# mjq11302010044/TPGSR

Hardware: AMD Instinct MI355X
Metric: training img/s (16x64->32x128, bs=48/GPU), TPGSR-TSRN full train step (higher is better)
Workload: dtype bf16x2; 1 GPU; C3: TPGSR-TSRN = TSRN_TL (STN+mask) + CRNN teacher/student text prior, stu_iter 1, full train step (teacher fwd, student fwd+bwd, distill loss, prior dropout, SR fwd+bwd, ImageLoss(gradient), clip 0.25, Adam); tpg=crnn, batch_per_gpu=48, global_batch=48, parallelism=dp1, launch=recorded plans, plain launches: main + weight-gradient + teacher streams

## Files before the change

include/tpgsr_hip.h:

```cpp
#ifndef TPGSR_HIP_H
#define TPGSR_HIP_H

#ifdef __cplusplus
extern "C" {
#endif

#define TPGSR_ACT_NONE 0
#define TPGSR_ACT_RELU 1
#define TPGSR_ACT_MISH 2
#define TPGSR_ACT_TANH 3
#define TPGSR_ACT_PRELU 4

const char* tpgsr_last_error(void);
int tpgsr_version(void);
int tpgsr_sizeof(int which);

typedef struct {
  const float* in;
  const float* in2;
  const float* in_scale;
  const float* in_shift;
  const float* wt;
  const float* bias;
  float* out;
// ... 252 lines not shown
  const float* dghn;
  const float* h;
  float* partC;
  float* dbC;
  float* partH;
  float* dbH;
  int axis;
  int zsplits;
} tpgsr_gru_wgrad_args;
int tpgsr_gru_wgrad_splits(long long P);
int tpgsr_gru_wgrad(const tpgsr_gru_wgrad_args* w, void* stream);
void tpgsr_gru_set_prefetch(int steps);

int tpgsr_tps_grid_fwd(const float* ctrl, const float* inv_kernel, const float* coord_repr, int N, int HW,
                       int NC, float* grid, float* src, void* stream);
int tpgsr_tps_grid_bwd(const float* dgrid, const float* src, const float* inv_kernel, const float* coord_repr,
                       int N, int HW, int NC, float* dctrl, void* stream);
int tpgsr_grid_sample_fwd(const float* in, const float* grid, int N, int H, int W, int C, int OH, int OW,
                          int align_corners, float* out, void* stream);
int tpgsr_grid_sample_bwd(const float* in, const float* grid, const float* dout, int N, int H, int W, int C,
                          int OH, int OW, int align_corners, float* din ,
                          float* dgrid , void* stream);

int tpgsr_strip_resample_fwd(const float* in, const float* scale, const float* shift, int act, int N, int Win, int Wout,
                             int C, float* out, void* stream);
int tpgsr_strip_resample_bwd(const float* in, const float* scale, const float* shift, int act, const float* dout, int N,
                             int Win, int Wout, int C, float* dz, void* stream);
int tpgsr_hsum(const float* d, int N, int H, int W, int C, float* dstrip, int accumulate, void* stream);

int tpgsr_bicubic_gray_fwd(const float* in_nchw, int N, int Ctot, int H, int W, int OH, int OW, float* out, void* stream);
int tpgsr_bicubic_gray_bwd(const float* dout, int N, int Ctot, int H, int W, int OH, int OW, float* din_nchw, void* stream);
int tpgsr_im2col3x3_c1(const float* in, int N, int H, int W, float* col , void* stream);
int tpgsr_col2im3x3_c1(const float* dcol, int N, int H, int W, float* din, void* stream);
int tpgsr_pad_channels(const float* src, long long M, int Cs, int Cd, float* dst, void* stream);
int tpgsr_pool2d_fwd(const float* x, int N, int H, int W, int C, const float* scale, const float* shift, int act, int KH,
                     int KW, int SH, int SW, int PH, int PW, float* out, void* stream);
int tpgsr_pool2d_bwd(const float* x, const float* dout, int N, int H, int W, int C, const float* scale, const float* shift,
                     int act, int KH, int KW, int SH, int SW, int PH, int PW, float* dz, void* stream);
int tpgsr_lstm_rec_gemm(const float* a0, const float* a1, long long a_stride, const float* b0, const float* b1, int Nrows,
                        int K, int Nc, int S, float* out, void* stream);
int tpgsr_lstm_step_fwd(float* G, const float* gh, int nsplit, const float* bhh , float* Cst, float* out,
                        int N, int T, int Hh, int step, void* stream);
int tpgsr_lstm_seq_fwd(float* G, const float* whhT, const float* bhh, float* Cst, float* out, void* hx, unsigned* sync, int N, int T,
                       int Hh, void* stream);
long long tpgsr_lstm_seq_hx_bytes(void);
int tpgsr_lstm_seq_probe(unsigned* words, void* stream);
int tpgsr_lstm_seq_fwdg(float* G, const float* whhT, const float* bhh, float* Cst, float* out, void* hg, unsigned* sync, int N, int T,
                        int Hh, void* stream);
long long tpgsr_lstm_seq_hg_bytes(void);
int tpgsr_lstm_seq_bwd(float* G, const float* Cst, const float* dout, const float* w0, const float* w1, void* px, unsigned* sync, int N,
                       int T, int Hh, void* stream);
long long tpgsr_lstm_seq_px_bytes(void);
int tpgsr_lstm_step_bwd(float* G, const float* Cst, const float* dout, const float* dhc, int nsplit, float* dcc, int N, int T,
                        int Hh, int step, void* stream);
int tpgsr_softmax_prior_fwd(const float* logits, const float* q, int N, int T, int C, int drop_n, float* p, float* prior_nchw,
                            float* partial, int nblk, void* stream);
int tpgsr_semantic_loss_finalize(const float* partial, int nblk, long long count, float w, float* loss, void* stream);
int tpgsr_softmax_prior_bwd(const float* p, const float* q, const float* dprior_nchw, const float* dp_in, int N, int T, int C,
                            int drop_n, float wsem, float* dlogits, int nblk, void* stream);
int tpgsr_ctc_loss(const float* logits, int sn, int st, const int* targets, const int* tgt_off, const int* tgt_len, const float* weight,
                   int N, int T, int C, int blank, float scale, float* nll, float* dlogits, int accumulate, int max_len, void* stream);
int tpgsr_semantic_loss_fwd(const float* p, const float* q, long long n, float* partial, int nblk, void* stream);
int tpgsr_semantic_loss_bwd(const float* p, const float* q, const float* dloss, long long n, float* dp, void* stream);

int tpgsr_copy_strided(const float* src, int src_ld, int src_coff, float* dst, int dst_ld, int dst_coff, long long M, int C,
                       int accumulate, void* stream);
// ... 98 lines not shown
```

tpgsr_amd/csrc/crnn.hip:

```cpp
#include "common.h"
#include "gru_common.h"
#include <stdlib.h>

__device__ __forceinline__ void cubic_coeffs(float t, float (&w)[4]) {
  const float A = -0.75f;
  float x = t + 1.f;
  w[0] = ((A * x - 5.f * A) * x + 8.f * A) * x - 4.f * A;
  x = t;
  w[1] = ((A + 2.f) * x - (A + 3.f)) * x * x + 1.f;
  x = 1.f - t;
  w[2] = ((A + 2.f) * x - (A + 3.f)) * x * x + 1.f;
  x = 2.f - t;
  w[3] = ((A * x - 5.f * A) * x + 8.f * A) * x - 4.f * A;
}

__device__ __forceinline__ void bicubic_src(int o, int in_size, int out_size, int& i0, float (&w)[4]) {
  float scale = (float)in_size / (float)out_size;
  float x = ((float)o + 0.5f) * scale - 0.5f;
  float fx = floorf(x);
  i0 = (int)fx;
  cubic_coeffs(x - fx, w);
}
__device__ __forceinline__ int clampi(int v, int lo, int hi) { return v < lo ? lo : (v > hi ? hi : v); }

// ... 412 lines not shown

extern "C" int tpgsr_pool2d_bwd(const float* x, const float* dout, int N, int H, int W, int C, const float* scale, const float* shift,
                                int act, int KH, int KW, int SH, int SW, int PH, int PW, float* dz, void* stream) {
  TPGSR_CHECK_ARG(x && dout && dz && KH > 0 && KW > 0 && SH > 0 && SW > 0, "tpgsr_pool2d_bwd: bad arguments");
  int OH = (H + 2 * PH - KH) / SH + 1, OW = (W + 2 * PW - KW) / SW + 1;
  const bool vec = (C & 3) == 0 && ((((uintptr_t)x | (uintptr_t)dout | (uintptr_t)dz) & 15) == 0);
  long long total = (long long)N * H * W * (vec ? C / 4 : C);
  TPGSR_CHECK_ARG((long long)N * H * W * C < (1ll << 31), "tpgsr_pool2d_bwd: map too large for the kernels' 32-bit indices");
  int grid = (int)min((long long)16384, (total + 255) / 256);
  static const bool fast2x2 = [] { const char* e = getenv("TPGSR_POOL2X2_FAST"); return !(e && e[0] == '0'); }();
  if (fast2x2 && vec && KH == 2 && KW == 2 && SH == 2 && SW == 2 && PH == 0 && PW == 0 && !(H & 1) && !(W & 1) &&
      (!scale || !(((uintptr_t)scale | (uintptr_t)shift) & 15))) {
    const long long tw = (long long)N * (H / 2) * (W / 2) * (C / 4);
    hipLaunchKernelGGL(pool2x2_bwd_kernel, dim3((int)min((long long)16384, (tw + 255) / 256)), dim3(256), 0, (hipStream_t)stream, x, dout, N, H, W,
                       C, scale, shift, act, dz);
    TPGSR_LAUNCH_CHECK("tpgsr_pool2d_bwd");
  }
  if (fast2x2 && vec && KH == 2 && KW == 2 && SH == 2 && SW == 1 && PH == 0 && PW == 1 && !(H & 1) &&
      (!scale || !(((uintptr_t)scale | (uintptr_t)shift) & 15))) {
    const long long tw = (long long)N * (H / 2) * W * (C / 4);
    hipLaunchKernelGGL(pool2x2s21_bwd_kernel, dim3((int)min((long long)16384, (tw + 255) / 256)), dim3(256), 0, (hipStream_t)stream, x, dout, N, H,
                       W, C, scale, shift, act, dz);
    TPGSR_LAUNCH_CHECK("tpgsr_pool2d_bwd");
  }
  if (vec)
    hipLaunchKernelGGL(pool2d_bwd_kernel<4>, dim3(grid), dim3(256), 0, (hipStream_t)stream, x, dout, N, H, W, C, scale, shift, act, KH, KW,
                       SH, SW, PH, PW, OH, OW, dz);
  else
    hipLaunchKernelGGL(pool2d_bwd_kernel<1>, dim3(grid), dim3(256), 0, (hipStream_t)stream, x, dout, N, H, W, C, scale, shift, act, KH, KW,
                       SH, SW, PH, PW, OH, OW, dz);
  TPGSR_LAUNCH_CHECK("tpgsr_pool2d_bwd");
}

#define RG_KC 32
__global__ __launch_bounds__(256) void lstm_rec_gemm_kernel(const float* __restrict__ a0, const float* __restrict__ a1,
                                                            long long a_stride, const float* __restrict__ b0,
                                                            const float* __restrict__ b1, int Nrows, int K, int Nc, int S,
                                                            float* __restrict__ out) {
  __shared__ float As[RG_KC][65];
  __shared__ float Bs[RG_KC][64];
  const int d = blockIdx.z, sp = blockIdx.y, n0 = blockIdx.x * 64;
  const float* A = d == 0 ? a0 : a1;
  const float* B = d == 0 ? b0 : b1;
  const int tid = threadIdx.x, lane = tid & 63, wave = tid >> 6;
  const int wm = wave & 1, wn = wave >> 1;
  const int kper = (K / RG_KC + S - 1) / S * RG_KC;
  const int kbeg = sp * kper, kend = min(K, kbeg + kper);
  const int aq = tid & 7, am0 = tid >> 3, bk0 = tid >> 4, bc = (tid & 15) * 4;
  floatx16 acc;
#pragma unroll
  for (int i = 0; i < 16; ++i) acc[i] = 0.f;
  const int arow = lane >> 5, acol = wm * 32 + (lane & 31), bcol = wn * 32 + (lane & 31);
  for (int k0 = kbeg; k0 < kend; k0 += RG_KC) {
    float4 ra0 = make_float4(0.f, 0.f, 0.f, 0.f), ra1 = ra0;
    const int k = k0 + aq * 4;
    if (am0 < Nrows && k < kend) ra0 = *reinterpret_cast<const float4*>(A + (size_t)am0 * a_stride + k);
    if (am0 + 32 < Nrows && k < kend) ra1 = *reinterpret_cast<const float4*>(A + (size_t)(am0 + 32) * a_stride + k);
    float4 rb0 = make_float4(0.f, 0.f, 0.f, 0.f), rb1 = rb0;
    if (k0 + bk0 < kend) rb0 = *reinterpret_cast<const float4*>(B + (size_t)(k0 + bk0) * Nc + n0 + bc);
    if (k0 + bk0 + 16 < kend) rb1 = *reinterpret_cast<const float4*>(B + (size_t)(k0 + bk0 + 16) * Nc + n0 + bc);
    __syncthreads();
    As[aq * 4 + 0][am0] = ra0.x; As[aq * 4 + 1][am0] = ra0.y; As[aq * 4 + 2][am0] = ra0.z; As[aq * 4 + 3][am0] = ra0.w;
    As[aq * 4 + 0][am0 + 32] = ra1.x; As[aq * 4 + 1][am0 + 32] = ra1.y; As[aq * 4 + 2][am0 + 32] = ra1.z; As[aq * 4 + 3][am0 + 32] = ra1.w;
    *reinterpret_cast<float4*>(&Bs[bk0][bc]) = rb0;
    *reinterpret_cast<float4*>(&Bs[bk0 + 16][bc]) = rb1;
    __syncthreads();
// ... 368 lines not shown
```

tpgsr_amd/csrc/plan.cpp:

```cpp
#include <hip/hip_runtime.h>
#include <string.h>
#include <memory>
#include <string>
#include <tuple>
#include <type_traits>
#include <unordered_map>
#include <utility>
#include <vector>
#include "../../include/tpgsr_hip.h"

void tpgsr_set_error(const char* fmt, ...);

namespace {

typedef int (*thunk_fn)(const tpgsr_plan_arg* a, void* stream);

template <typename T>
inline T arg_as(const tpgsr_plan_arg& a) {
  if constexpr (std::is_pointer<T>::value) return reinterpret_cast<T>(const_cast<void*>(a.p));
  else if constexpr (std::is_floating_point<T>::value) return static_cast<T>(a.f);
  else return static_cast<T>(a.i);
}

template <typename Tuple, typename F, size_t... I>
// ... 13 lines not shown
    return call_with<Tuple>(fn, a, st, std::make_index_sequence<sizeof...(P) - 1>{});
  }
};

struct Entry {
  thunk_fn fn;
  int nargs;
  int struct_bytes;
};

#define TPGSR_REG(sym) {#sym, {&Thunk<decltype(&sym), &sym>::call, Thunk<decltype(&sym), &sym>::nargs, 0}}
#define TPGSR_REG_S(sym, T) {#sym, {&Thunk<decltype(&sym), &sym>::call, Thunk<decltype(&sym), &sym>::nargs, (int)sizeof(T)}}

const std::unordered_map<std::string, Entry>& registry() {
  static const std::unordered_map<std::string, Entry> r = {
      TPGSR_REG_S(tpgsr_conv_fwd, tpgsr_conv_args), TPGSR_REG_S(tpgsr_conv_wgrad, tpgsr_wgrad_args),
      TPGSR_REG(tpgsr_wgrad_reduce), TPGSR_REG(tpgsr_wgrad_reduce_program), TPGSR_REG(tpgsr_conv_wgrad_batch), TPGSR_REG(tpgsr_compose_bwd_program), TPGSR_REG(tpgsr_pack_conv_weight), TPGSR_REG(tpgsr_pack_tail_weight),
      TPGSR_REG(tpgsr_pack_program), TPGSR_REG(tpgsr_mfma_probe), TPGSR_REG(tpgsr_copy), TPGSR_REG(tpgsr_zero),
      TPGSR_REG(tpgsr_bn_finalize), TPGSR_REG(tpgsr_bn_stats), TPGSR_REG(tpgsr_bn_bwd_reduce),
      TPGSR_REG(tpgsr_bn_bwd_finalize), TPGSR_REG(tpgsr_bn_bwd_apply), TPGSR_REG(tpgsr_affine_act),
      TPGSR_REG(tpgsr_affine_act_pool), TPGSR_REG(tpgsr_affine_act_pool_bwd), TPGSR_REG(tpgsr_prelu_fwd),
      TPGSR_REG(tpgsr_prelu_bwd), TPGSR_REG(tpgsr_add), TPGSR_REG(tpgsr_add_n), TPGSR_REG(tpgsr_act_bwd), TPGSR_REG(tpgsr_nchw_to_nhwc),
      TPGSR_REG(tpgsr_nhwc_to_nchw), TPGSR_REG(tpgsr_reduce_partials), TPGSR_REG(tpgsr_bigru_fwd),
      TPGSR_REG(tpgsr_bigru_bwd), TPGSR_REG(tpgsr_bigru_bwd2), TPGSR_REG(tpgsr_bigru_fwd_u), TPGSR_REG(tpgsr_bigru_bwd_u), TPGSR_REG_S(tpgsr_bigru_proj_fwd, tpgsr_bigru_proj_args), TPGSR_REG_S(tpgsr_gru_wgrad, tpgsr_gru_wgrad_args), TPGSR_REG(tpgsr_tps_grid_fwd), TPGSR_REG(tpgsr_tps_grid_bwd),
      TPGSR_REG(tpgsr_grid_sample_fwd), TPGSR_REG(tpgsr_grid_sample_bwd), TPGSR_REG(tpgsr_strip_resample_fwd),
      TPGSR_REG(tpgsr_strip_resample_bwd), TPGSR_REG(tpgsr_hsum), TPGSR_REG(tpgsr_bicubic_gray_fwd),
      TPGSR_REG(tpgsr_bicubic_gray_bwd), TPGSR_REG(tpgsr_pool2d_fwd), TPGSR_REG(tpgsr_pool2d_bwd),
      TPGSR_REG(tpgsr_lstm_rec_gemm), TPGSR_REG(tpgsr_lstm_step_fwd), TPGSR_REG(tpgsr_lstm_seq_fwd), TPGSR_REG(tpgsr_lstm_seq_fwdg), TPGSR_REG(tpgsr_lstm_seq_bwd), TPGSR_REG(tpgsr_lstm_step_bwd), TPGSR_REG(tpgsr_softmax_prior_fwd),
      TPGSR_REG(tpgsr_semantic_loss_finalize), TPGSR_REG(tpgsr_softmax_prior_bwd), TPGSR_REG(tpgsr_tail_shiftsum_tanh), TPGSR_REG(tpgsr_shiftsum_nhwc),
      TPGSR_REG(tpgsr_tail_bwd), TPGSR_REG(tpgsr_image_loss_fwd), TPGSR_REG(tpgsr_image_loss_finalize),
      TPGSR_REG(tpgsr_image_loss_bwd), TPGSR_REG(tpgsr_l1_loss_fwd), TPGSR_REG(tpgsr_l1_loss_bwd), TPGSR_REG(tpgsr_sumsq_partial), TPGSR_REG(tpgsr_clip_coef),
      TPGSR_REG(tpgsr_adam_step), TPGSR_REG(tpgsr_step_inc), TPGSR_REG(tpgsr_scale_),
      TPGSR_REG(tpgsr_im2col3x3_c1), TPGSR_REG(tpgsr_col2im3x3_c1), TPGSR_REG(tpgsr_pad_channels),
      TPGSR_REG(tpgsr_semantic_loss_fwd), TPGSR_REG(tpgsr_semantic_loss_bwd), TPGSR_REG(tpgsr_split_bf_program),
      TPGSR_REG(tpgsr_copy_strided), TPGSR_REG(tpgsr_resize_nearest_fwd), TPGSR_REG(tpgsr_resize_nearest_bwd), TPGSR_REG(tpgsr_resize_bilinear_fwd),
      TPGSR_REG(tpgsr_resize_bilinear_bwd), TPGSR_REG(tpgsr_dilate2d), TPGSR_REG(tpgsr_subsample2d), TPGSR_REG(tpgsr_hreduce), TPGSR_REG(tpgsr_hbroadcast),
      TPGSR_REG(tpgsr_bicubic_upsample),
      TPGSR_REG(tpgsr_tconv4s2_expand), TPGSR_REG(tpgsr_tconv4s2_fold_grad), TPGSR_REG(tpgsr_tconv4s2_small_fwd),
      TPGSR_REG(tpgsr_tconv4s2_small_bwd_data), TPGSR_REG(tpgsr_tconv4s2_small_bwd_weight), TPGSR_REG(tpgsr_leaky_relu_fwd),
      TPGSR_REG(tpgsr_leaky_relu_bwd), TPGSR_REG(tpgsr_charbonnier_loss_fwd), TPGSR_REG(tpgsr_charbonnier_loss_bwd),
      TPGSR_REG(tpgsr_leaky_relu_window), TPGSR_REG(tpgsr_scaled_add), TPGSR_REG(tpgsr_dense_bwd_step),
      TPGSR_REG(tpgsr_conv3x3_narrow_fwd), TPGSR_REG(tpgsr_conv3x3_narrow_bwd_data), TPGSR_REG(tpgsr_conv3x3_narrow_bwd_weight),
  };
  return r;
}

enum { OP_LAUNCH = 0, OP_FORK = 1, OP_JOIN = 2, OP_EDGE = 3 };
constexpr int MAX_ARGS = 24;

struct Op {
  int kind, sid, nargs;
  thunk_fn fn;
  const char* name;
  tpgsr_plan_arg args[MAX_ARGS];
  int blob;
  hipEvent_t ev;
};

struct Plan {
  std::vector<Op> ops;
  std::vector<std::unique_ptr<char[]>> blobs;
  std::vector<hipEvent_t> stamps;
  std::vector<void*> stamp_stream;
  bool stamped = false;
  ~Plan() {
    for (auto& o : ops)
// ... 300 lines not shown
```

tpgsr_amd/engine_crnn.py:

```python
from __future__ import annotations

import os
from typing import Optional

import torch

from . import kernels as K
from .engine import BNLayer, ConvLayer, F32, _EngineBase
from .kernels import ConvGeom, Plan, recording


class Conv0Im2col:

    def __init__(self, eng, wname, bname):
        self.eng, self.wname, self.bname = eng, wname, bname
        self.w, self.b = eng.P[wname], eng.P[bname]
        assert tuple(self.w.shape[1:]) == (1, 3, 3)
        self.Cout, self.Cin = self.w.shape[0], 12
        dev = eng.device
        self.wt_f = torch.zeros(12, self.Cout, dtype=F32, device=dev)
        self.wt_d = torch.zeros(self.Cout, 12, dtype=F32, device=dev)
        eng.add_pack(self.w, self.wt_f, self.wt_d, Cout=self.Cout, Cin=9, KH=1, KW=1, kind=0, f_ld=self.Cout, d_ld=12)
        eng.register_operand(self.wt_f, self.wt_d)

    def fwd(self, N, H, W, gray, col, out, **kw):
        K.im2col3x3_c1(gray, N, H, W, col)
        K.conv_fwd(K.make_conv_args(ConvGeom(N, H, W, 12, self.Cout), col, self.wt_f, out, bias=self.b, **kw))

    def wgrad(self, N, H, W, col, dy):
        eng, g = self.eng, ConvGeom(N, H, W, 12, self.Cout)
        Z = K.wgrad_splits(g.M, g.K, g.Cout)
        part, dbp = eng.wgrad_buffers(Z * g.K * g.Cout, Z * g.Cout)
        with K.side():
            K.conv_wgrad(K.make_wgrad_args(K.make_conv_args(g, col), dy, part, dbp))
            K.wgrad_reduce(part, dbp, Z, g, eng.G[self.wname], eng.G[self.bname], accumulate=True, real=(9, 1, 1, 0))

    def dgrad(self, N, H, W, dy, dcol, dgray):
        K.conv_fwd(K.make_conv_args(ConvGeom(N, H, W, self.Cout, 12), dy, self.wt_d, dcol))
        K.col2im3x3_c1(dcol, N, H, W, dgray)


class PaddedLinear:

    def __init__(self, eng, wname, bname):
        self.eng, self.wname, self.bname = eng, wname, bname
        self.w, self.b = eng.P[wname], eng.P[bname]
        self.Cout, self.Cin = self.w.shape
        self.Cp = (self.Cout + 3) // 4 * 4
        dev = eng.device
        self.wt_f = torch.zeros(self.Cin, self.Cp, dtype=F32, device=dev)
        self.wt_d = torch.zeros(self.Cp, self.Cin, dtype=F32, device=dev)
        eng.add_pack(self.w, self.wt_f, self.wt_d, Cout=self.Cout, Cin=self.Cin, kind=0, f_ld=self.Cp)
        eng.register_operand(self.wt_f, self.wt_d)

    def fwd(self, N, H, W, x, out, **kw):
        K.conv_fwd(K.make_conv_args(ConvGeom(N, H, W, self.Cin, self.Cout), x, self.wt_f, out, bias=self.b, wt_ld=self.Cp, **kw))

    def dgrad(self, N, H, W, dy_p, dx):
        K.conv_fwd(K.make_conv_args(ConvGeom(N, H, W, self.Cp, self.Cin), dy_p, self.wt_d, dx))

    def wgrad(self, N, H, W, x, dy_p):
        eng, g = self.eng, ConvGeom(N, H, W, self.Cin, self.Cout)
        Z = K.wgrad_splits(g.M, g.K, g.Cout)
        part, dbp = eng.wgrad_buffers(Z * g.K * g.Cout, Z * g.Cout)
        with K.side():
            K.conv_wgrad(K.make_wgrad_args(K.make_conv_args(g, x), dy_p, part, dbp, dy_ld=self.Cp))
            K.wgrad_reduce(part, dbp, Z, g, eng.G[self.wname], eng.G[self.bname], accumulate=True)


class LstmLayer:
    MAX_BATCH = 64

# ... 92 lines not shown
                one(ge, K.make_conv_args(ge, out), de, Gd[emb.wname], Gd[emb.bname],
                    **(dict(dy_ld=emb.Cp) if isinstance(emb, PaddedLinear) else {}))
            for d, suf in enumerate(("", "_reverse")):
                sgn = 1 if d == 0 else -1
                gh_ = ConvGeom(N, 1, T, Hh, G4, 1, 1, 0, sgn, 1, T)
                one(gh_, K.make_conv_args(gh_, out, in_ld=2 * Hh, in_coff=d * Hh), G, Gd[r + "weight_hh_l0" + suf], Gd[r + "bias_hh_l0" + suf],
                    dy_ld=2 * G4, dy_coff=d * G4)
                gi_ = ConvGeom(N, 1, T, self.Cin, G4)
                one(gi_, K.make_conv_args(gi_, x, **loader), G, Gd[r + "weight_ih_l0" + suf], Gd[r + "bias_ih_l0" + suf],
                    dy_ld=2 * G4, dy_coff=d * G4)
            if batch:
                K.conv_wgrad_batch(wargs)
                for part, dbp, Z, g_, dw_, db_ in reduces:
                    K.wgrad_reduce(part, dbp, Z, g_, dw_, db_, accumulate=True)
        if dx is not None:
            K.conv_fwd(K.make_conv_args(ConvGeom(N, 1, T, 2 * G4, self.Cin), G, self.wih_d, dx, bnb=dx_bnb))


class CRNNEngine(_EngineBase):
    IMG_HW = (32, 100)
    POOLS = {0: ((2, 2), (2, 2), (0, 0)), 1: ((2, 2), (2, 2), (0, 0)), 3: ((2, 2), (2, 1), (0, 1)), 5: ((2, 2), (2, 1), (0, 1))}
    BN_AT = (2, 4, 6)
    EARLY_CONVS = 3

    def __init__(self, module: torch.nn.Module):
        super().__init__(module)
        env = os.environ.get
        self.overlap_wgrad = env("TPGSR_OVERLAP_WGRAD", "1") != "0"
        self.defer_reduce = env("TPGSR_DEFER_REDUCE", "1") != "0"
        self.pack_split = env("TPGSR_CRNN_PACK_SPLIT", "1") != "0"
        self.early_reduce = env("TPGSR_CRNN_EARLY_REDUCE", "1") != "0"
        self.bwd_split = env("TPGSR_CRNN_BWD_SPLIT", "1") != "0"
        self.side_batch = int(env("TPGSR_SIDE_BATCH_CRNN", "0"))

    def _build_layers(self):
        self.convs, self.bns = [], {}
        for i in range(7):
            k, pad = (3, 1) if i < 6 else (2, 0)
            self._pack_group = 0 if i < self.EARLY_CONVS else 1
            if i == 0:
                self.convs.append(Conv0Im2col(self, "cnn.conv0.weight", "cnn.conv0.bias"))
            else:
                self.convs.append(ConvLayer(self, f"cnn.conv{i}.weight", f"cnn.conv{i}.bias", k, k, pad, pad, need_dgrad=True))
            if i in self.BN_AT:
                self.bns[i] = BNLayer(self, f"cnn.batchnorm{i}")
        self.lstm = [LstmLayer(self, "rnn.0"), LstmLayer(self, "rnn.1")]
        self._pack_group = 0
        self.nclass = self.P["rnn.1.embedding.weight"].shape[0]

    def _dims(self):
        h, w = self.IMG_HW
        dims = []
        for i in range(7):
            k, pad = (3, 1) if i < 6 else (2, 0)
            oh, ow = h + 2 * pad - k + 1, w + 2 * pad - k + 1
            ph, pw = oh, ow
            if i in self.POOLS:
                (kh, kw), (sh, sw), (pdh, pdw) = self.POOLS[i]
                ph, pw = (oh + 2 * pdh - kh) // sh + 1, (ow + 2 * pdw - kw) // sw + 1
            dims.append(((h, w), (oh, ow), (ph, pw)))
            h, w = ph, pw
        assert h == 1, "the height of conv must be 1"
        return dims

    def plans(self, N, training, slot=0):
        return self._two_pass((N, bool(training), slot, getattr(self, "role", "tpg"), K.POLICY), lambda ws, final: self._record(N, training, ws, final))

    def _record(self, N, training, ws, final):
        fwd, dgp, pack = Plan("crnn_fwd"), Plan("crnn_dgray"), Plan("crnn_pack")
        fwd_b, pack_late = Plan("crnn_fwd_b"), Plan("crnn_pack_late")
        bwd, bwd_b = (K.backward_plan(n, overlap=self.overlap_wgrad, defer=self.defer_reduce) for n in ("crnn_bwd", "crnn_bwd_b"))
        fwd.final = bwd.final = bwd_b.final = dgp.final = pack.final = fwd_b.final = pack_late.final = final
        split_pack = training and self.pack_split
        self._cur_ws, self._wg_idx = ws, 0
        for bn in self._bn_layers:
            bn.use(ws)
        if not training:
            with recording(pack):
                self.pack_all()
        if split_pack:
            with recording(pack_late):
                self.pack_group(1)
        with recording(fwd), K.conv_terms(K.terms_for(getattr(self, "role", "tpg"), "fwd")):
            self._record_fwd(N, training, ws, cut_to=fwd_b if split_pack else None)
        if training:
            with recording(bwd), K.conv_terms(K.terms_for("tpg", "bwd")):
                self._record_bwd(N, ws, cut_to=bwd_b if self.bwd_split else None)
                if self.defer_reduce:
                    K.flush_wgrad_reduces()
                K._REC.join()
            with recording(dgp), K.conv_terms(K.terms_for("tpg", "bwd")):
                self._record_dgray(N, ws)
        out = dict(fwd=fwd, bwd=bwd, dgray=dgp, pack=pack, ws=ws)
        if len(bwd_b):
            out["bwd_b"] = bwd_b
        if split_pack:
            out["fwd_b"], out["pack_late"] = fwd_b, pack_late
        return out

    def _record_fwd(self, N, training, ws, cut_to=None):
        if training:
            if cut_to is not None:
                self.pack_group(0)
            else:
                self.pack_all()
        dims = self._dims()
        cur, loader = K.DynPtr("gray"), {}
        for i, conv in enumerate(self.convs):
            if cut_to is not None and i == self.EARLY_CONVS:
                K.continue_in(cut_to)
            (h, w), (oh, ow), (ph, pw) = dims[i]
            s = ws(f"s{i}", N * oh * ow, conv.Cout)
            bn = self.bns.get(i)
            part = bn.partial(N * oh * ow)[0] if (bn and training) else None
            if i == 0:
                conv.fwd(N, h, w, cur, ws("col0", N * h * w, 12), s)
            else:
                conv.fwd(N, h, w, cur, s, bn_partial=part, **loader)
            if bn:
                bn.finalize(N * oh * ow, conv.b, training)
            if i in self.POOLS:
                k, st, pd = self.POOLS[i]
                a = ws(f"a{i}", N * ph * pw, conv.Cout)
                K.pool2d_fwd(s, N, oh, ow, conv.Cout, bn.scale if bn else None, bn.shift if bn else None, "relu", k, st, pd, a)
                cur, loader = a, {}
            else:
                cur, loader = s, (dict(in_act="relu", **bn.loader) if bn else dict(in_act="relu"))
        T = dims[6][1][1]
        self.T = T
        x = cur
        for j, L in enumerate(self.lstm):
            G4 = 4 * L.Hh
            G = ws(f"l{j}_G", N * T, 2 * G4)
            gh = ws(f"l{j}_gh", L.Hh // 32, 2, N, G4)
            Cst = ws(f"l{j}_C", N * T, 2 * L.Hh)
            out = ws(f"l{j}_out", N * T, 2 * L.Hh)
            e = ws(f"l{j}_e", N * T, L.emb.Cout)
            L.fwd(N, T, x, G, gh, Cst, out, e, **(loader if j == 0 else {}))
            x = e
        K.copy(x, K.DynPtr("logits"), N * T * self.nclass)

    def _record_bwd(self, N, ws, cut_to=None):
        t = ws.t
        dims = self._dims()
        T = self.T
        cp = self.lstm[1].emb.Cp if isinstance(self.lstm[1].emb, PaddedLinear) else self.nclass
        de = ws("dlogits", N * T, cp)
        K.pad_channels(K.DynPtr("dlogits"), N * T, self.nclass, cp, de)
        cnn_loader = dict(in_act="relu", **self.bns[6].loader)
        fz = None
        sbl = self.side_batch
        sb = K.side_batch_begin() if sbl >= 1 else False
        for j in (1, 0):
            L = self.lstm[j]
            G4 = 4 * L.Hh
            dout = ws(f"l{j}_dout", N * T, 2 * L.Hh)
            dhc = ws(f"l{j}_dhc", 4 * L.Hh // 32, 2, N, L.Hh)
            dcc = ws(f"l{j}_dcc", N, 2 * L.Hh)
            x = t[f"l{j - 1}_e"] if j == 1 else t["s6"]
            dx = ws(f"l{j}_dx", N * T, L.Cin)
            if j == 0:
                fz = self.bns[6].fuse_stats(t["s6"], N * T, "relu", 2 * G4)
            L.bwd(N, T, x, t[f"l{j}_G"], t[f"l{j}_C"], t[f"l{j}_out"], de, dout, dhc, dcc, dx, dx_bnb=fz, **({} if j == 1 else cnn_loader))
            de = dx
        da = de
        K.side_batch_end(sb)
        sb = False
        for i in range(6, -1, -1):
            conv, bn = self.convs[i], self.bns.get(i)
            if not sb and (sbl >= 1 and i == 6 or sbl >= 2 and i == 2):
                sb = K.side_batch_begin()
            (h, w), (oh, ow), (ph, pw) = dims[i]
            M = N * oh * ow
            s = t[f"s{i}"]
            ds = ws(f"ds{i}", M, conv.Cout)
            if i in self.POOLS:
                k, st, pd = self.POOLS[i]
                K.pool2d_bwd(s, da, N, oh, ow, conv.Cout, bn.scale if bn else None, bn.shift if bn else None, "relu", k, st, pd, ds)
                if bn:
                    dz = ds
                    ds = ws(f"ds{i}b", M, conv.Cout)
                    bn.backward(dz, None, s, M, "none", ds)
            elif bn:
                bn.backward(da, None, s, M, "relu", ds, fused=fz)
            else:
                K.act_bwd(s, da, M * conv.Cout, "relu", ds)
            if i == 0:
                K.side_batch_end(sb)
                conv.wgrad(N, h, w, t["col0"], ds)
                continue
            else:
                pi, pbn = i - 1, self.bns.get(i - 1)
                if pi in self.POOLS:
                    xin, ld = t[f"a{pi}"], {}
                else:
                    xin, ld = t[f"s{pi}"], (dict(in_act="relu", **pbn.loader) if pbn else dict(in_act="relu"))
            conv.wgrad(N, h, w, xin, ds, loader=ld)
            if i == 3 and self.defer_reduce and self.early_reduce:
                K.flush_wgrad_reduces()
                K.side_batch_end(sb)
                sb = False
                if cut_to is not None:
                    K.continue_in(cut_to)
            da = ws(f"da{i - 1}", N * h * w, conv.Cin)
            fz = pbn.fuse_stats(t[f"s{pi}"], N * h * w, "relu", conv.Cout) if (pbn and pi not in self.POOLS) else None
            conv.dgrad(N, h, w, ds, da, **(dict(bnb=fz) if fz else {}))

    def _record_dgray(self, N, ws):
        h, w = self.IMG_HW
        dcol = ws("dcol0", N * h * w, 12)
        self.convs[0].dgrad(N, h, w, ws.t["ds0"], dcol, K.DynPtr("dgray"))

    def forward(self, gray: torch.Tensor, training: bool, slot: int = 0, late_stream=None, after_late=None) -> torch.Tensor:
        if not gray.is_cuda and not K.DRYRUN:
            raise RuntimeError("tpgsr_amd runs on the GPU only (no CPU fallback): move the module and inputs to cuda")
        if gray.dim() != 4 or gray.shape[1] != 1 or tuple(gray.shape[2:]) != self.IMG_HW:
            raise ValueError(f"CRNN expects (N, 1, {self.IMG_HW[0]}, {self.IMG_HW[1]}) input, got {tuple(gray.shape)}")
        LstmLayer.check_batch(gray.shape[0])
        self.bind(gray.device)
        N = gray.shape[0]
        pl = self.plans(N, training, slot)
        gray = gray.contiguous().float()
        logits = torch.empty(N, self.T, self.nclass, dtype=F32, device=gray.device)
        fwd = pl["fwd"]
        fwd.set_ptr("gray", gray.data_ptr())
        if "fwd_b" in pl:
            cur, ev = K.current_stream(), None
            if late_stream is not None and late_stream is not cur:
                K.order(late_stream, cur)
                with K.stream_ctx(late_stream):
                    pl["pack_late"].run()
                ev = K.event_record(late_stream)
            else:
                pl["pack_late"].run()
            if after_late is not None:
                after_late()
            fwd.run()
            K.event_wait(cur, ev)
            pl["fwd_b"].set_ptr("logits", logits.data_ptr())
            pl["fwd_b"].run()
        else:
            if after_late is not None:
                after_late()
            fwd.set_ptr("logits", logits.data_ptr())
            if not training:
                self.pack_if_stale(pl["pack"])
            fwd.run()
        if training:
            self.note_packed()
            self._pending_batches += 1
        self._last_gray = gray
        return logits

    EARLY_FINAL_FROM = "cnn.conv3.weight"

    def early_final_offset(self) -> Optional[int]:
        if not (self.defer_reduce and self.early_reduce and self.bwd_split):
            return None
        return self.arena.layout()[0][self.EARLY_FINAL_FROM]

    def backward(self, N, gray: torch.Tensor, dlogits: torch.Tensor, need_dgray: bool = False, slot: int = 0,
                 after_early=None) -> Optional[torch.Tensor]:
        pl = self.plans(N, True, slot)
        self.arena.attach_grads()
        bwd = pl["bwd"]
        dlogits = dlogits.contiguous().float()
        bwd.set_ptr("dlogits", dlogits.data_ptr())
        bwd.run()
        if "bwd_b" in pl:
            if after_early is not None:
                after_early()
            pl["bwd_b"].run()
        if not need_dgray:
            return None
        dgray = torch.empty_like(gray)
        pl["dgray"].set_ptr("dgray", dgray.data_ptr())
        pl["dgray"].run()
        return dgray
```

tpgsr_amd/kernels.py:

```python
from __future__ import annotations

import ctypes as C
import os
from dataclasses import dataclass
from typing import Optional

import torch

from . import _lib
from ._lib import ConvArgs, GruWgradArgs, WgradArgs, act_code, check


DRYRUN = os.environ.get("TPGSR_PLAN_DRYRUN") == "1"


_TERMS = {"f32": 0, "x3": 3, "bf16": 1, "x2": 2, "x3b2": 3}
_X2_TPG_FWD = int(os.environ.get("TPGSR_X2_TPG_FWD", "3"))
POLICY = os.environ.get("TPGSR_CONV_PREC", "x3")
if POLICY not in _TERMS:
    raise ValueError(f"TPGSR_CONV_PREC={POLICY!r}: expected one of {sorted(_TERMS)}")
CONV_TERMS = _TERMS[POLICY]


_POLICY_EXPLICIT = "TPGSR_CONV_PREC" in os.environ
# ... 1144 lines not shown
def sumsq_partial(x, n, partial, nblk):
    _launch("tpgsr_sumsq_partial", _p(x), n, _p(partial), nblk)


def clip_coef(partial, nblk, max_norm, coef, norm_out=None):
    _launch("tpgsr_clip_coef", _p(partial), nblk, max_norm, _p(coef), _p(norm_out))


def adam_step(p, g, m, v, n, gscale, lr, beta1, beta2, eps, step_dev):
    _launch("tpgsr_adam_step", _p(p), _p(g), _p(m), _p(v), n, _p(gscale), lr, beta1, beta2, eps, _p(step_dev))


def step_inc(step_dev):
    _launch("tpgsr_step_inc", _p(step_dev))


def clip_coef_steps(partial, nblk, max_norm, coef, norm_out, step_devs):
    arr = (C.c_void_p * max(1, len(step_devs)))(*[t.data_ptr() for t in step_devs])
    _launch("tpgsr_clip_coef_steps", _p(partial), nblk, max_norm, _p(coef), _p(norm_out), C.cast(arr, C.c_void_p), len(step_devs))


def scale_(x, n, coef):
    _launch("tpgsr_scale_", _p(x), n, _p(coef))


def im2col3x3_c1(inp, N, H, W, col):
    _launch("tpgsr_im2col3x3_c1", _p(inp), N, H, W, _p(col))


def col2im3x3_c1(dcol, N, H, W, din):
    _launch("tpgsr_col2im3x3_c1", _p(dcol), N, H, W, _p(din))


def pad_channels(src, M, Cs, Cd, dst):
    _launch("tpgsr_pad_channels", _p(src), M, Cs, Cd, _p(dst))


def semantic_loss_fwd(p, q, n, partial, nblk):
    _launch("tpgsr_semantic_loss_fwd", _p(p), _p(q), n, _p(partial), nblk)


def semantic_loss_bwd(p, q, dloss, n, dp):
    _launch("tpgsr_semantic_loss_bwd", _p(p), _p(q), _p(dloss), n, _p(dp))


def make_bf_twin(wt: torch.Tensor, cin: int = 0):
    lib = _lib.load()
    Kd, N = wt.shape
    cin = block_order_cin(Kd, cin)
    kp = (Kd + 31) // 32 * 32
    twin = torch.zeros(3 * ((N + 31) // 32 * 32) * kp, dtype=torch.bfloat16, device=wt.device)
    d = (_lib.SplitDesc * 1)()
    d[0].src, d[0].dst, d[0].K, d[0].N, d[0].ld, d[0].kp, d[0].blk0, d[0].cin = wt.data_ptr(), twin.data_ptr(), Kd, N, N, kp, 0, cin
    table = torch.frombuffer(bytearray(bytes(d)), dtype=torch.uint8).to(wt.device)
    split_bf_program(table, 1, lib.tpgsr_split_bf_blocks(Kd, N))
    register_bf_twin(wt, twin, kp, cin)
    return twin, kp


def split_bf_program(descs_dev, ndesc, total_blocks):
    _launch("tpgsr_split_bf_program", _p(descs_dev), ndesc, total_blocks)


def copy_strided(src, src_ld, src_coff, dst, dst_ld, dst_coff, M, C_, accumulate=False):
    _launch("tpgsr_copy_strided", _p(src), src_ld, src_coff, _p(dst), dst_ld, dst_coff, M, C_, int(accumulate))

# ... 175 lines not shown
```

tpgsr_amd/model/crnn/crnn.py:

```python
import weakref

import torch
from torch import nn

from ..nn_params import BatchNormParams, Conv2dParams, EngineHolder, LinearParams, LSTMParams, _NoForward


class BidirectionalLSTM(_NoForward):
    def __init__(self, nIn, nHidden, nOut):
        super().__init__()
        self.rnn = LSTMParams(nIn, nHidden, bidirectional=True)
        self.embedding = LinearParams(nHidden * 2, nOut)


class _CRNNFunction(torch.autograd.Function):
    @staticmethod
    def forward(ctx, gray, anchor, net):
        eng = net._engine()
        eng.bind(gray.device)
        ctx.slot, ctx.gen = eng.acquire_slot() if net.training else (0, 0)
        if net.training:
            weakref.finalize(ctx, eng.release_slot, ctx.slot, ctx.gen)
        logits = eng.forward(gray, net.training, slot=ctx.slot)
        ctx.net, ctx.mode, ctx.N = net, net.training, gray.shape[0]
        ctx.save_for_backward(gray.contiguous().float())
        ctx.need_dgray = gray.requires_grad
        return logits.permute(1, 0, 2)

    @staticmethod
    def backward(ctx, dlogits_tnc):
        if not ctx.mode:
            raise RuntimeError("backward through an eval-mode CRNN forward is not supported")
        (gray,) = ctx.saved_tensors
        eng = ctx.net._engine()
        eng.check_slot(ctx.slot, ctx.gen)
        dgray = eng.backward(ctx.N, gray, dlogits_tnc.permute(1, 0, 2).contiguous(), ctx.need_dgray, slot=ctx.slot)
        eng.release_slot(ctx.slot, ctx.gen)
        sync = getattr(ctx.net, "_grad_sync", None)
        if sync is not None:
            sync(eng)
        return dgray, None, None


class CRNN(EngineHolder, nn.Module):

    def __init__(self, imgH, nc, nclass, nh, n_rnn=2, leakyRelu=False):
        super().__init__()
        assert imgH % 16 == 0, "imgH has to be a multiple of 16"
        if leakyRelu or nc != 1 or imgH != 32:
            raise NotImplementedError("the TPGSR path uses CRNN(32, 1, 37, 256) with ReLU (interfaces/base.py:635)")
        ks = [3, 3, 3, 3, 3, 3, 2]
        ps = [1, 1, 1, 1, 1, 1, 0]
        nm = [64, 128, 256, 256, 512, 512, 512]
        cnn = nn.Sequential()
        for i in range(7):
            n_in = nc if i == 0 else nm[i - 1]
# ... 33 lines not shown
```

Measured before the change: 8868 img/s.

## Fuse CRNN conv0 weight-gradient with ReLU/pool backward when input gradient is unneeded

```diff
diff --git a/include/tpgsr_hip.h b/include/tpgsr_hip.h
--- a/include/tpgsr_hip.h
+++ b/include/tpgsr_hip.h
@@ -308,6 +308,10 @@
 int tpgsr_bicubic_gray_bwd(const float* dout, int N, int Ctot, int H, int W, int OH, int OW, float* din_nchw, void* stream);
 int tpgsr_im2col3x3_c1(const float* in, int N, int H, int W, float* col , void* stream);
 int tpgsr_col2im3x3_c1(const float* dcol, int N, int H, int W, float* din, void* stream);
+int tpgsr_conv0_relu_pool_fwd(const float* gray, const float* w, const float* b, int N, int H, int W, int Cout,
+                              float* s_out , float* a_out, void* stream);
+int tpgsr_conv0_relu_pool_bwd(const float* gray, const float* s, const float* da, int N, int H, int W, int Cout,
+                              float* ds_out , float* part, int nblk, void* stream);
 int tpgsr_pad_channels(const float* src, long long M, int Cs, int Cd, float* dst, void* stream);
 int tpgsr_pool2d_fwd(const float* x, int N, int H, int W, int C, const float* scale, const float* shift, int act, int KH,
                      int KW, int SH, int SW, int PH, int PW, float* out, void* stream);
diff --git a/tpgsr_amd/csrc/crnn.hip b/tpgsr_amd/csrc/crnn.hip
--- a/tpgsr_amd/csrc/crnn.hip
+++ b/tpgsr_amd/csrc/crnn.hip
@@ -468,6 +468,188 @@
   TPGSR_LAUNCH_CHECK("tpgsr_pool2d_bwd");
 }
 
+namespace {
+
+constexpr int kC0Threads = 256;
+constexpr int kC0MaxCout = 1024;
+constexpr int kC0Acc = 40;
+
+struct C0Window {
+  int n, oh, ow;
+};
+
+__device__ __forceinline__ C0Window c0_window(unsigned wi, int OH, int OW) {
+  const unsigned r = wi / (unsigned)OW;
+  C0Window q;
+  q.ow = (int)(wi - r * OW);
+  q.n = (int)(r / (unsigned)OH);
+  q.oh = (int)(r - (unsigned)q.n * OH);
+  return q;
+}
+
+__device__ __forceinline__ void c0_patch(const float* __restrict__ gray, const C0Window& q, int H, int W, float (&patch)[4][4]) {
+  const float* g = gray + (size_t)q.n * H * W;
+#pragma unroll
+  for (int a = 0; a < 4; ++a) {
+    const int y = 2 * q.oh - 1 + a;
+#pragma unroll
+    for (int b = 0; b < 4; ++b) {
+      const int x = 2 * q.ow - 1 + b;
+      patch[a][b] = ((unsigned)y < (unsigned)H && (unsigned)x < (unsigned)W) ? g[(size_t)y * W + x] : 0.f;
+    }
+  }
+}
+
+__global__ __launch_bounds__(kC0Threads) void conv0_relu_pool_fwd_kernel(const float* __restrict__ gray, const float* __restrict__ w,
+                                                                         const float* __restrict__ b, int N, int H, int W, int Cout,
+                                                                         float* __restrict__ s_out, float* __restrict__ a_out, int wvec) {
+  const int Q = Cout >> 2, WL = kC0Threads / Q, OH = H >> 1, OW = W >> 1;
+  const int wl = threadIdx.x / Q, c = (threadIdx.x - wl * Q) * 4;
+  if (wl >= WL) return;
+  float wr[4][9], br[4];
+  if (wvec) {
+    const float4* w4 = reinterpret_cast<const float4*>(w + (size_t)c * 9);
+#pragma unroll
+    for (int k = 0; k < 9; ++k) {
+      const float4 t = w4[k];
+      (&wr[0][0])[4 * k] = t.x; (&wr[0][0])[4 * k + 1] = t.y; (&wr[0][0])[4 * k + 2] = t.z; (&wr[0][0])[4 * k + 3] = t.w;
+    }
+  } else {
+#pragma unroll
+    for (int k = 0; k < 36; ++k) (&wr[0][0])[k] = w[(size_t)c * 9 + k];
+  }
+#pragma unroll
+  for (int v = 0; v < 4; ++v) br[v] = b[c + v];
+  const unsigned total = (unsigned)N * OH * OW;
+  for (unsigned wi = blockIdx.x * WL + wl; wi < total; wi += gridDim.x * WL) {
+    const C0Window q = c0_window(wi, OH, OW);
+    float patch[4][4];
+    c0_patch(gray, q, H, W, patch);
+    float best[4] = {-INFINITY, -INFINITY, -INFINITY, -INFINITY};
+#pragma unroll
+    for (int py = 0; py < 2; ++py)
+#pragma unroll
+      for (int px = 0; px < 2; ++px) {
+        float acc[4];
+#pragma unroll
+        for (int v = 0; v < 4; ++v) {
+          acc[v] = br[v];
+#pragma unroll
+          for (int kh = 0; kh < 3; ++kh)
+#pragma unroll
+            for (int kw = 0; kw < 3; ++kw) acc[v] = __builtin_fmaf(wr[v][kh * 3 + kw], patch[py + kh][px + kw], acc[v]);
+          const float val = fmaxf(acc[v], 0.f);
+          if (val > best[v] || val != val) best[v] = val;
+        }
+        if (s_out)
+          *reinterpret_cast<float4*>(s_out + ((size_t)(q.n * H + 2 * q.oh + py) * W + 2 * q.ow + px) * Cout + c) =
+              make_float4(acc[0], acc[1], acc[2], acc[3]);
+      }
+    *reinterpret_cast<float4*>(a_out + (size_t)wi * Cout + c) = make_float4(best[0], best[1], best[2], best[3]);
+  }
+}
+
+__global__ __launch_bounds__(kC0Threads) void conv0_relu_pool_bwd_kernel(const float* __restrict__ gray, const float* __restrict__ s,
+                                                                         const float* __restrict__ da, int N, int H, int W, int Cout,
+                                                                         float* __restrict__ ds_out, float* __restrict__ part) {
+  __shared__ float red[kC0Threads][kC0Acc + 1];
+  const int Q = Cout >> 2, WL = kC0Threads / Q, OH = H >> 1, OW = W >> 1;
+  const int wl = threadIdx.x / Q, c = (threadIdx.x - wl * Q) * 4;
+  float acc[4][9], accb[4];
+#pragma unroll
+  for (int v = 0; v < 4; ++v) {
+    accb[v] = 0.f;
+#pragma unroll
+    for (int k = 0; k < 9; ++k) acc[v][k] = 0.f;
+  }
+  const unsigned total = (unsigned)N * OH * OW;
+  if (wl < WL)
+    for (unsigned wi = blockIdx.x * WL + wl; wi < total; wi += gridDim.x * WL) {
+      const C0Window q = c0_window(wi, OH, OW);
+      const size_t base = ((size_t)(q.n * H + 2 * q.oh) * W + 2 * q.ow) * Cout + c;
+      const size_t offs[4] = {0, (size_t)Cout, (size_t)W * Cout, (size_t)W * Cout + Cout};
+      float4 sv4[4];
+#pragma unroll
+      for (int k = 0; k < 4; ++k) sv4[k] = *reinterpret_cast<const float4*>(s + base + offs[k]);
+      const float4 g4 = *reinterpret_cast<const float4*>(da + (size_t)wi * Cout + c);
+      float patch[4][4];
+      c0_patch(gray, q, H, W, patch);
+      const float sv[4][4] = {{sv4[0].x, sv4[1].x, sv4[2].x, sv4[3].x}, {sv4[0].y, sv4[1].y, sv4[2].y, sv4[3].y},
+                              {sv4[0].z, sv4[1].z, sv4[2].z, sv4[3].z}, {sv4[0].w, sv4[1].w, sv4[2].w, sv4[3].w}};
+      const float gv[4] = {g4.x, g4.y, g4.z, g4.w};
+      float d[4][4];
+#pragma unroll
+      for (int v = 0; v < 4; ++v) {
+        int k = 0;
+        float bestv = fmaxf(sv[v][0], 0.f);
+#pragma unroll
+        for (int j = 1; j < 4; ++j) {
+          const float val = fmaxf(sv[v][j], 0.f);
+          if (val > bestv) { bestv = val; k = j; }
+        }
+#pragma unroll
+        for (int j = 0; j < 4; ++j) {
+          d[j][v] = k == j ? gv[v] * (sv[v][j] > 0.f ? 1.f : 0.f) : 0.f;
+          accb[v] += d[j][v];
+#pragma unroll
+          for (int kh = 0; kh < 3; ++kh)
+#pragma unroll
+            for (int kw = 0; kw < 3; ++kw) acc[v][kh * 3 + kw] = __builtin_fmaf(d[j][v], patch[(j >> 1) + kh][(j & 1) + kw], acc[v][kh * 3 + kw]);
+        }
+      }
+      if (ds_out) {
+#pragma unroll
+        for (int j = 0; j < 4; ++j) *reinterpret_cast<float4*>(ds_out + base + offs[j]) = make_float4(d[j][0], d[j][1], d[j][2], d[j][3]);
+      }
+    }
+#pragma unroll
+  for (int e = 0; e < 36; ++e) red[threadIdx.x][e] = (&acc[0][0])[e];
+#pragma unroll
+  for (int v = 0; v < 4; ++v) red[threadIdx.x][36 + v] = accb[v];
+  __syncthreads();
+  float* row = part + (size_t)blockIdx.x * Cout * 10;
+  for (int o = threadIdx.x; o < Q * kC0Acc; o += kC0Threads) {
+    const int qd = o / kC0Acc, e = o - qd * kC0Acc;
+    float sum = 0.f;
+    for (int l = 0; l < WL; ++l) sum += red[l * Q + qd][e];
+    row[e < 36 ? qd * 36 + e : Cout * 9 + qd * 4 + (e - 36)] = sum;
+  }
+}
+
+inline bool conv0_args_ok(int N, int H, int W, int Cout) {
+  return N > 0 && H > 0 && W > 0 && !(H & 1) && !(W & 1) && Cout >= 4 && !(Cout & 3) && Cout <= kC0MaxCout &&
+         (long long)N * H * W * Cout < (1ll << 31);
+}
+#define CONV0_ARGS_MSG ": needs even H and W, Cout a multiple of 4 (<= 1024) and N H W Cout < 2^31, got N %d, H %d, W %d, Cout %d"
+
+inline int conv0_grid(int N, int H, int W, int Cout, int cap) {
+  const int WL = kC0Threads / (Cout >> 2);
+  const long long windows = (long long)N * (H >> 1) * (W >> 1);
+  return (int)min((long long)cap, (windows + WL - 1) / WL);
+}
+
+}
+
+extern "C" int tpgsr_conv0_relu_pool_fwd(const float* gray, const float* w, const float* b, int N, int H, int W, int Cout, float* s_out,
+                                         float* a_out, void* stream) {
+  TPGSR_CHECK_ARG(gray && w && b && a_out, "tpgsr_conv0_relu_pool_fwd: null pointer");
+  TPGSR_CHECK_ARG(conv0_args_ok(N, H, W, Cout), "tpgsr_conv0_relu_pool_fwd" CONV0_ARGS_MSG, N, H, W, Cout);
+  TPGSR_CHECK_ARG((((uintptr_t)s_out | (uintptr_t)a_out) & 15) == 0, "tpgsr_conv0_relu_pool_fwd: s_out / a_out must be 16-byte aligned");
+  hipLaunchKernelGGL(conv0_relu_pool_fwd_kernel, dim3((conv0_grid(N, H, W, Cout, 1 << 20) + 1) / 2), dim3(kC0Threads), 0, (hipStream_t)stream,
+                     gray, w, b, N, H, W, Cout, s_out, a_out, ((uintptr_t)w & 15) == 0 ? 1 : 0);
+  TPGSR_LAUNCH_CHECK("tpgsr_conv0_relu_pool_fwd");
+}
+
+extern "C" int tpgsr_conv0_relu_pool_bwd(const float* gray, const float* s, const float* da, int N, int H, int W, int Cout, float* ds_out,
+                                         float* part, int nblk, void* stream) {
+  TPGSR_CHECK_ARG(gray && s && da && part, "tpgsr_conv0_relu_pool_bwd: null pointer");
+  TPGSR_CHECK_ARG(conv0_args_ok(N, H, W, Cout), "tpgsr_conv0_relu_pool_bwd" CONV0_ARGS_MSG, N, H, W, Cout);
+  TPGSR_CHECK_ARG(nblk > 0 && nblk <= 65536, "tpgsr_conv0_relu_pool_bwd: 1 <= nblk <= 65536 rows of partial sums, got %d", nblk);
+  TPGSR_CHECK_ARG((((uintptr_t)s | (uintptr_t)da | (uintptr_t)ds_out) & 15) == 0, "tpgsr_conv0_relu_pool_bwd: s / da / ds_out must be 16-byte aligned");
+  hipLaunchKernelGGL(conv0_relu_pool_bwd_kernel, dim3(nblk), dim3(kC0Threads), 0, (hipStream_t)stream, gray, s, da, N, H, W, Cout, ds_out, part);
+  TPGSR_LAUNCH_CHECK("tpgsr_conv0_relu_pool_bwd");
+}
+
 #define RG_KC 32
 __global__ __launch_bounds__(256) void lstm_rec_gemm_kernel(const float* __restrict__ a0, const float* __restrict__ a1,
                                                             long long a_stride, const float* __restrict__ b0,
diff --git a/tpgsr_amd/csrc/plan.cpp b/tpgsr_amd/csrc/plan.cpp
--- a/tpgsr_amd/csrc/plan.cpp
+++ b/tpgsr_amd/csrc/plan.cpp
@@ -69,6 +69,7 @@
       TPGSR_REG(tpgsr_image_loss_bwd), TPGSR_REG(tpgsr_l1_loss_fwd), TPGSR_REG(tpgsr_l1_loss_bwd), TPGSR_REG(tpgsr_sumsq_partial), TPGSR_REG(tpgsr_clip_coef),
       TPGSR_REG(tpgsr_adam_step), TPGSR_REG(tpgsr_step_inc), TPGSR_REG(tpgsr_scale_),
       TPGSR_REG(tpgsr_im2col3x3_c1), TPGSR_REG(tpgsr_col2im3x3_c1), TPGSR_REG(tpgsr_pad_channels),
+      TPGSR_REG(tpgsr_conv0_relu_pool_fwd), TPGSR_REG(tpgsr_conv0_relu_pool_bwd),
       TPGSR_REG(tpgsr_semantic_loss_fwd), TPGSR_REG(tpgsr_semantic_loss_bwd), TPGSR_REG(tpgsr_split_bf_program),
       TPGSR_REG(tpgsr_copy_strided), TPGSR_REG(tpgsr_resize_nearest_fwd), TPGSR_REG(tpgsr_resize_nearest_bwd), TPGSR_REG(tpgsr_resize_bilinear_fwd),
       TPGSR_REG(tpgsr_resize_bilinear_bwd), TPGSR_REG(tpgsr_dilate2d), TPGSR_REG(tpgsr_subsample2d), TPGSR_REG(tpgsr_hreduce), TPGSR_REG(tpgsr_hbroadcast),
diff --git a/tpgsr_amd/engine_crnn.py b/tpgsr_amd/engine_crnn.py
--- a/tpgsr_amd/engine_crnn.py
+++ b/tpgsr_amd/engine_crnn.py
@@ -38,6 +38,24 @@
     def dgrad(self, N, H, W, dy, dcol, dgray):
         K.conv_fwd(K.make_conv_args(ConvGeom(N, H, W, self.Cout, 12), dy, self.wt_d, dcol))
         K.col2im3x3_c1(dcol, N, H, W, dgray)
+
+
+class Conv0Direct:
+
+    def __init__(self, eng, wname, bname):
+        self.eng, self.wname, self.bname = eng, wname, bname
+        assert tuple(eng.P[wname].shape[1:]) == (1, 3, 3)
+        self.Cout = eng.P[wname].shape[0]
+
+    def bwd(self, N, H, W, gray, s, da):
+        eng, C = self.eng, self.Cout
+        nblk = K.conv0_bwd_blocks(N, H, W, C)
+        part = eng.wgrad_buffers(nblk * C * 10)[0]
+        o = eng.arena.offsets[self.wname]
+        assert eng.arena.offsets[self.bname] == o + C * 9, f"{self.bname} does not follow {self.wname} in the gradient arena"
+        with K.side():
+            K.conv0_relu_pool_bwd(gray, s, da, N, H, W, C, None, part, nblk)
+            K.reduce_partials(part, nblk, C * 10, eng.arena.grad[o:o + C * 10], accumulate=True)
 
 
 class PaddedLinear:
@@ -196,6 +214,7 @@
         self.early_reduce = env("TPGSR_CRNN_EARLY_REDUCE", "1") != "0"
         self.bwd_split = env("TPGSR_CRNN_BWD_SPLIT", "1") != "0"
         self.side_batch = int(env("TPGSR_SIDE_BATCH_CRNN", "0"))
+        self._dgray_of = {}
 
     def _build_layers(self):
         self.convs, self.bns = [], {}
@@ -204,6 +223,7 @@
             self._pack_group = 0 if i < self.EARLY_CONVS else 1
             if i == 0:
                 self.convs.append(Conv0Im2col(self, "cnn.conv0.weight", "cnn.conv0.bias"))
+                self.conv0_direct = Conv0Direct(self, "cnn.conv0.weight", "cnn.conv0.bias")
             else:
                 self.convs.append(ConvLayer(self, f"cnn.conv{i}.weight", f"cnn.conv{i}.bias", k, k, pad, pad, need_dgrad=True))
             if i in self.BN_AT:
@@ -227,10 +247,12 @@
         assert h == 1, "the height of conv must be 1"
         return dims
 
-    def plans(self, N, training, slot=0):
-        return self._two_pass((N, bool(training), slot, getattr(self, "role", "tpg"), K.POLICY), lambda ws, final: self._record(N, training, ws, final))
-
-    def _record(self, N, training, ws, final):
+    def plans(self, N, training, slot=0, dgray=True):
+        key = (N, bool(training), slot, getattr(self, "role", "tpg"), K.POLICY)
+        dgray = bool(dgray or not training)
+        return self._two_pass(key if dgray else key + ("no d gray",), lambda ws, final: self._record(N, training, ws, final, dgray))
+
+    def _record(self, N, training, ws, final, dgray=True):
         fwd, dgp, pack = Plan("crnn_fwd"), Plan("crnn_dgray"), Plan("crnn_pack")
         fwd_b, pack_late = Plan("crnn_fwd_b"), Plan("crnn_pack_late")
         bwd, bwd_b = (K.backward_plan(n, overlap=self.overlap_wgrad, defer=self.defer_reduce) for n in ("crnn_bwd", "crnn_bwd_b"))
@@ -249,12 +271,13 @@
             self._record_fwd(N, training, ws, cut_to=fwd_b if split_pack else None)
         if training:
             with recording(bwd), K.conv_terms(K.terms_for("tpg", "bwd")):
-                self._record_bwd(N, ws, cut_to=bwd_b if self.bwd_split else None)
+                self._record_bwd(N, ws, cut_to=bwd_b if self.bwd_split else None, dgray=dgray)
                 if self.defer_reduce:
                     K.flush_wgrad_reduces()
                 K._REC.join()
-            with recording(dgp), K.conv_terms(K.terms_for("tpg", "bwd")):
-                self._record_dgray(N, ws)
+            if dgray:
+                with recording(dgp), K.conv_terms(K.terms_for("tpg", "bwd")):
+                    self._record_dgray(N, ws)
         out = dict(fwd=fwd, bwd=bwd, dgray=dgp, pack=pack, ws=ws)
         if len(bwd_b):
             out["bwd_b"] = bwd_b
@@ -304,7 +327,7 @@
             x = e
         K.copy(x, K.DynPtr("logits"), N * T * self.nclass)
 
-    def _record_bwd(self, N, ws, cut_to=None):
+    def _record_bwd(self, N, ws, cut_to=None, dgray=True):
         t = ws.t
         dims = self._dims()
         T = self.T
@@ -337,6 +360,10 @@
             (h, w), (oh, ow), (ph, pw) = dims[i]
             M = N * oh * ow
             s = t[f"s{i}"]
+            if i == 0 and not dgray:
+                K.side_batch_end(sb)
+                self.conv0_direct.bwd(N, h, w, K.DynPtr("gray"), s, da)
+                continue
             ds = ws(f"ds{i}", M, conv.Cout)
             if i in self.POOLS:
                 k, st, pd = self.POOLS[i]
@@ -375,7 +402,8 @@
         dcol = ws("dcol0", N * h * w, 12)
         self.convs[0].dgrad(N, h, w, ws.t["ds0"], dcol, K.DynPtr("dgray"))
 
-    def forward(self, gray: torch.Tensor, training: bool, slot: int = 0, late_stream=None, after_late=None) -> torch.Tensor:
+    def forward(self, gray: torch.Tensor, training: bool, slot: int = 0, late_stream=None, after_late=None,
+                need_dgray: Optional[bool] = None) -> torch.Tensor:
         if not gray.is_cuda and not K.DRYRUN:
             raise RuntimeError("tpgsr_amd runs on the GPU only (no CPU fallback): move the module and inputs to cuda")
         if gray.dim() != 4 or gray.shape[1] != 1 or tuple(gray.shape[2:]) != self.IMG_HW:
@@ -383,7 +411,10 @@
         LstmLayer.check_batch(gray.shape[0])
         self.bind(gray.device)
         N = gray.shape[0]
-        pl = self.plans(N, training, slot)
+        dgray = bool(slot > 0 if need_dgray is None else need_dgray)
+        if training:
+            self._dgray_of[(N, slot)] = dgray
+        pl = self.plans(N, training, slot, dgray)
         gray = gray.contiguous().float()
         logits = torch.empty(N, self.T, self.nclass, dtype=F32, device=gray.device)
         fwd = pl["fwd"]
@@ -425,11 +456,18 @@
 
     def backward(self, N, gray: torch.Tensor, dlogits: torch.Tensor, need_dgray: bool = False, slot: int = 0,
                  after_early=None) -> Optional[torch.Tensor]:
-        pl = self.plans(N, True, slot)
+        dgray_plan = self._dgray_of.get((N, slot), True)
+        if need_dgray and not dgray_plan:
+            raise RuntimeError("CRNNEngine.backward: d gray was not announced to the forward pass of this slot (forward(..., need_dgray=True)): "
+                               "its backward plan keeps no ds0")
+        pl = self.plans(N, True, slot, dgray_plan)
         self.arena.attach_grads()
         bwd = pl["bwd"]
         dlogits = dlogits.contiguous().float()
         bwd.set_ptr("dlogits", dlogits.data_ptr())
+        if not dgray_plan:
+            gray = gray.contiguous().float()
+            pl.get("bwd_b", bwd).set_ptr("gray", gray.data_ptr())
         bwd.run()
         if "bwd_b" in pl:
             if after_early is not None:
diff --git a/tpgsr_amd/kernels.py b/tpgsr_amd/kernels.py
--- a/tpgsr_amd/kernels.py
+++ b/tpgsr_amd/kernels.py
@@ -1200,6 +1200,42 @@
     _launch("tpgsr_col2im3x3_c1", _p(dcol), N, H, W, _p(din))
 
 
+CONV0_BWD_BLOCKS = 768
+
+
+def conv0_bwd_blocks(N, H, W, Cout) -> int:
+    wl = 256 // max(1, Cout // 4)
+    groups = max(1, -(-(N * (H // 2) * (W // 2)) // max(1, wl)))
+    iters = -(-groups // CONV0_BWD_BLOCKS)
+    return -(-groups // iters)
+
+
+def _conv0_check(who, N, H, W, Cout, gray, a, s=None, w=None, b=None):
+    if min(N, H, W) < 1 or H % 2 or W % 2:
+        raise ValueError(f"{who}: needs even H and W (2x2 pooling windows), got N {N}, H {H}, W {W}")
+    if Cout % 4 or not 4 <= Cout <= 1024:
+        raise ValueError(f"{who}: takes an output channel count that is a multiple of 4 up to 1024, got {Cout}")
+    if N * H * W * Cout >= 1 << 31:
+        raise ValueError(f"{who}: needs N H W Cout < 2^31 (32-bit indices), got {N} x {H} x {W} x {Cout}")
+    sizes = ((gray, N * H * W), (a, N * H * W * Cout // 4), (s, N * H * W * Cout), (w, Cout * 9), (b, Cout))
+    if any(t is not None and not isinstance(t, (int, DynPtr)) and t.numel() != n for t, n in sizes):
+        raise ValueError(f"{who}: tensor sizes do not match N {N}, H {H}, W {W}, Cout {Cout}")
+
+
+def conv0_relu_pool_fwd(gray, w, b, N, H, W, Cout, s_out, a_out):
+    _conv0_check("conv0_relu_pool_fwd", N, H, W, Cout, gray, a_out, s_out, w, b)
+    _launch("tpgsr_conv0_relu_pool_fwd", _p(gray), _p(w), _p(b), N, H, W, Cout, _p(s_out), _p(a_out))
+
+
+def conv0_relu_pool_bwd(gray, s, da, N, H, W, Cout, ds_out, part, nblk):
+    _conv0_check("conv0_relu_pool_bwd", N, H, W, Cout, gray, da, s)
+    if ds_out is not None and ds_out.numel() != N * H * W * Cout:
+        raise ValueError(f"conv0_relu_pool_bwd: ds_out holds {ds_out.numel()} floats, expected {N * H * W * Cout}")
+    if not 1 <= nblk <= 65536 or part.numel() < nblk * Cout * 10:
+        raise ValueError(f"conv0_relu_pool_bwd: partial holds {part.numel()} floats, {nblk} workgroups write {nblk * Cout * 10}")
+    _launch("tpgsr_conv0_relu_pool_bwd", _p(gray), _p(s), _p(da), N, H, W, Cout, _p(ds_out), _p(part), nblk)
+
+
 def pad_channels(src, M, Cs, Cd, dst):
     _launch("tpgsr_pad_channels", _p(src), M, Cs, Cd, _p(dst))
 
diff --git a/tpgsr_amd/model/crnn/crnn.py b/tpgsr_amd/model/crnn/crnn.py
--- a/tpgsr_amd/model/crnn/crnn.py
+++ b/tpgsr_amd/model/crnn/crnn.py
@@ -21,7 +21,7 @@
         ctx.slot, ctx.gen = eng.acquire_slot() if net.training else (0, 0)
         if net.training:
             weakref.finalize(ctx, eng.release_slot, ctx.slot, ctx.gen)
-        logits = eng.forward(gray, net.training, slot=ctx.slot)
+        logits = eng.forward(gray, net.training, slot=ctx.slot, need_dgray=gray.requires_grad)
         ctx.net, ctx.mode, ctx.N = net, net.training, gray.shape[0]
         ctx.save_for_backward(gray.contiguous().float())
         ctx.need_dgray = gray.requires_grad
```

Result: no change. 8916 img/s, median of 6 (+0.6%).
